# MatchaChoco010/toy-cpu-pathtracing

Measured on AMD Instinct MI355X. Metric: Msamples/sec (whole node), scene3 MIS/Sobol 1920x1080, higher is better.
Workload: dtype f32; 1 GPU; scene3 1920x1080 mis+sobol, 1024-spp job, 1024 sample indices per step (BASELINE configs[1]); parallelism=single-gpu

## Files before the change

toy-cpu-pathtracing_amd/csrc/api.cpp:

```cpp
#include <cstring>

#include "api_internal.hpp"

using namespace pt;

static thread_local std::string g_err;
bool pt::g_debug_unlocked = false;
int pt::fail(int code, const std::string& msg) { g_err = msg; return code; }

static const uint32_t CIE_CMF_BITS[470 * 4] = {
#include "cie_cmf.inc"
};
void pt::cie_cmf4(float out[470 * 4]) { std::memcpy(out, CIE_CMF_BITS, sizeof(CIE_CMF_BITS)); }

int pt::get_launch_ctx(const mi355pt_scene* sc, uint32_t seed, LaunchCtx** out, int* slot) {
    if (sc->ctx && sc->ctx->device != sc->impl.device) {
        delete sc->ctx; sc->ctx = nullptr;
    }
    if (!sc->ctx) {
        LaunchCtx* lc = new LaunchCtx();
        lc->device = sc->impl.device;
        HIP_TRY(hipMalloc((void**)&lc->d_hash, sizeof(uint64_t) * HASH_TABLE_DIMS));
        HIP_TRY(hipMalloc((void**)&lc->d_counters, sizeof(unsigned) * CTX_RING));
        HIP_TRY(hipMalloc((void**)&lc->d_stats, sizeof(DevStats) * CTX_RING));
// ... 78 lines not shown
    if (hipGetDevice(&dev) != hipSuccess || dev != s->impl.device)
        return fail(MI355PT_E_DEVICE, "current HIP device is not the device the scene was built on");
    return MI355PT_OK;
}

static int launch_range(const mi355pt_scene* s, const mi355pt_camera* cam, const mi355pt_params* p, uint32_t s_begin, uint32_t s_end, float* d_accum,
                        hipStream_t stream, mi355pt_stats* stats, const PathOut& pout, int aov_kind, uint32_t illuminant_lut, const uint32_t* d_list,
                        uint32_t n_list) {
    const bool aov = aov_kind >= 0;
    if (!d_list && shard_tile_count(cam->width, cam->height, p->shard_index, p->shard_count) == 0) return MI355PT_OK;
    int rc;
    LaunchCtx* lc; int slot;
    if ((rc = get_launch_ctx(s, p->seed, &lc, &slot))) return rc;
    if (lc->device != s->impl.device) return fail(MI355PT_E_DEVICE, "launch context and scene live on different devices");
    const bool want_stats = stats && p->collect_stats;
    int& waves = aov ? lc->aov_waves[aov_kind] : lc->waves[want_stats ? 1 : 0][p->sampler & 1u][p->strategy < 3u ? p->strategy : 0u];
    if (!waves) waves = aov ? query_resident_waves_aov((uint32_t)aov_kind, s->impl.features)
                            : query_resident_waves(select_kernel(false, want_stats, s->impl.features, p->sampler, p->strategy));
    const DevCamera dc = make_camera(cam);
    LaunchPlan plan = d_list ? plan_launch_tiles(cam, p, s_begin, s_end, waves, n_list) : plan_launch(cam, p, s_begin, s_end, waves, aov);
    DevParams& dp = plan.params;
    if (d_list) set_tile_list(dp, d_list);
    dp.stats_mode = p->collect_stats;
    return timed_launch(lc, slot, stream, stats, want_stats || aov, [&](unsigned* d_counter, DevStats* d_stats) {
        if ((rc = grow_device_buffer(&lc->d_partial, &lc->partial_bytes, plan.partial_floats * sizeof(float), stream))) return rc;
        const KernelKey key = select_kernel(d_list != nullptr, want_stats, s->impl.features, p->sampler, p->strategy);
        if ((rc = grow_device_buffer(&lc->d_defer, &lc->defer_bytes, aov ? (size_t)0 : query_defer_bytes_per_wave(key) * (size_t)plan.grid, stream))) return rc;
        if (aov) HIP_TRY(launch_aov((uint32_t)aov_kind, s->impl.dev, dc, dp, illuminant_lut, lc->d_hash, d_accum, d_counter, stats ? d_stats : nullptr,
                                    s->impl.features, plan.grid, stream));
        else {
            DevScene dev = s->impl.dev;
            dev.cam_lists = use_camera_lists(key, dp.block_log2, camera_lists_enabled()) ? 1u : 0u;
            dev.queue_stage = use_queue_staging(key, queue_staging_enabled()) ? 1u : 0u;
            dev.light_queue = use_light_queue(key, light_queue_enabled()) ? 1u : 0u;
            HIP_TRY(launch_pt(key, dev, dc, dp, plan.n_tiles,
                              lc->d_hash, d_accum, lc->d_partial, d_counter, d_list ? nullptr : d_stats, plan.grid, stream, pout, lc->d_defer));
        }
        return (int)MI355PT_OK;
    });
}

int pt::launch_ranges(const mi355pt_scene* s, const mi355pt_camera* cam, const mi355pt_params* p, uint32_t s_begin, uint32_t s_end, float* d_accum,
                      hipStream_t stream, mi355pt_stats* stats, const uint32_t* d_list, uint32_t n_list, const PathOut& pout, int aov_kind,
                      uint32_t illuminant_lut) {
    return for_each_launch_range(p->sampler, stats != nullptr, s_begin, s_end, [&](uint32_t b, uint32_t e) {
        return launch_range(s, cam, p, b, e, d_accum, stream, stats, pout, aov_kind, illuminant_lut, d_list, n_list);
    });
}

int pt::render_accum_range(const mi355pt_scene* s, const mi355pt_camera* cam, const mi355pt_params* p, uint32_t s_begin, uint32_t s_end,
                           float* d_accum, void* hip_stream, mi355pt_stats* stats, const PathOut& pout, int aov_kind, uint32_t illuminant_lut) {
    const bool aov = aov_kind >= 0;
    int rc = check_args(s, cam, p, aov);
    if (rc) return rc;
    if (!d_accum || s_end > p->spp || s_begin >= s_end) return fail(MI355PT_E_INVALID, "bad sample range or null accumulator");
    if (aov) {
        if (aov_kind > MI355PT_AOV_SHADING_NORMAL) return fail(MI355PT_E_INVALID, "unknown AOV kind");
        if (p->collect_stats) return fail(MI355PT_E_INVALID, "the AOV renderers have no instrumented kernel: collect_stats must be 0");
        if (aov_kind == MI355PT_AOV_ALBEDO && illuminant_lut >= s->impl.luts.size())
// ... 95 lines not shown
```

toy-cpu-pathtracing_amd/csrc/launch_plan.hpp:

```cpp
#pragma once
#include <algorithm>
#include <cmath>
#include <cstddef>
#include <cstdint>
#include <cstdlib>

#include "../../include/mi355pt.h"
#include "layout.hpp"

namespace pt {

struct V3 { float x, y, z; };
inline V3 cross3(V3 a, V3 b) { return {a.y * b.z - b.y * a.z, a.z * b.x - b.z * a.x, a.x * b.y - b.x * a.y}; }
inline V3 norm3(V3 a) { float r = 1.0f / std::sqrt((a.x * a.x) + (a.y * a.y) + (a.z * a.z)); return {a.x * r, a.y * r, a.z * r}; }

inline uint32_t log2_int(uint32_t v) { return v == 0 ? 0 : 31 - (uint32_t)__builtin_clz(v); }
inline uint32_t round_up_pow2(uint32_t v) { return v <= 1 ? 1 : 1u << (32 - __builtin_clz(v - 1)); }

inline uint32_t shard_tile_count(uint32_t width, uint32_t height, uint32_t shard_index, uint32_t shard_count) {
    const uint32_t total = ((width + 7) / 8) * ((height + 7) / 8);
    const uint32_t cnt = shard_count ? shard_count : 1u, idx = shard_count ? shard_index : 0u;
    return total > idx ? (total - idx + cnt - 1) / cnt : 0u;
}

// ... 136 lines not shown
#undef PT_SET_ENTRY
inline uint32_t pick_features(uint32_t feat) {
    for (uint32_t s : FEATURE_SETS) if ((feat & ~s) == 0u) return s;
    return FEAT_ALL;
}
struct KernelKey { bool tiles, stats; uint32_t mode, set; };
inline KernelKey select_kernel(bool tiles, bool stats, uint32_t feat, uint32_t sampler, uint32_t strategy) {
    if (stats) return KernelKey{tiles, true, MODE_GENERIC, (feat & (FEAT_CC | FEAT_EMTEX)) == 0u ? FEAT_STD & ~FEAT_CC : FEAT_ALL};
    const uint32_t mode = sampler == MI355PT_SAMPLER_SOBOL && strategy == MI355PT_STRATEGY_MIS ? MODE_MIS_SOBOL
                        : sampler == MI355PT_SAMPLER_SOBOL && strategy == MI355PT_STRATEGY_NEE ? MODE_NEE_SOBOL
                        : strategy == MI355PT_STRATEGY_PT ? MODE_PT : MODE_GENERIC;
    return KernelKey{tiles, false, mode, pick_features(feat)};
}

inline bool use_camera_lists(const KernelKey& key, uint32_t block_log2, bool enabled) { return enabled && !key.stats && block_log2 <= 3u; }
inline bool camera_lists_enabled() { const char* e = getenv("MI355PT_NO_CAMERA_LISTS"); return !(e && e[0] != '\0' && !(e[0] == '0' && e[1] == '\0')); }

inline bool use_queue_staging(const KernelKey& key, bool enabled) { return enabled && !key.stats; }
inline bool queue_staging_enabled() { const char* e = getenv("MI355PT_NO_QUEUE_STAGING"); return !(e && e[0] != '\0' && !(e[0] == '0' && e[1] == '\0')); }

inline bool use_light_queue(const KernelKey& key, bool enabled) { return enabled && !key.stats; }
inline bool light_queue_enabled() { const char* e = getenv("MI355PT_NO_LIGHT_QUEUE"); return !(e && e[0] != '\0' && !(e[0] == '0' && e[1] == '\0')); }

}
```

toy-cpu-pathtracing_amd/csrc/layout.hpp:

```cpp
#pragma once
#include <stddef.h>
#include <stdint.h>

#if defined(__HIPCC__)
#define PT_HD __host__ __device__
#else
#define PT_HD
#endif

namespace pt {

#ifndef PT_STACK_DEPTH
#define PT_STACK_DEPTH 24
#endif
constexpr int STACK_DEPTH = PT_STACK_DEPTH;
constexpr int MAX_LEAF_TRIS = 4;
constexpr int MAX_BUILD_DEPTH = 22;
constexpr int HASH_TABLE_DIMS = 136;

struct alignas(16) DevNode {
    float bx[4];
    float by[4];
    float bz[4];
    int32_t child[2];
// ... 139 lines not shown
    const DevTri* tris_render;
    float tri_shift[3]; uint32_t tris_are_local;
    float shared_mw[3]; uint32_t pad_mw;
    const DevInstance* instances;
    const DevMaterial* materials;
    const DevLight* lights;
    const DevLightTri* light_tris;
    const float* light_uvs;
    const float* luts;
    const float* cmf;
    const float* rgb2spec;
    const float* z_nodes;
    const uint32_t* texels;
    const DevTexture* textures;
    const float* cc_albedo;
    uint32_t n_nodes, n_tris, n_lights, n_materials;
    int32_t root;
    int32_t root4;
    uint32_t n_nodes4;
    uint32_t cam_lists;
    const DevEnv* envs;
    uint32_t n_envs;
    uint16_t queue_stage;
    uint16_t light_queue;
};

struct DevCamera {
    float s[3], u[3], f[3];
    float tan_half_fov, aspect;
    uint32_t width, height;
};

struct DevParams {
    uint32_t spp, seed, max_depth, strategy, sampler;
    float exposure;
    uint32_t log2_spp, n_base4_digits;
    uint32_t sample_begin, sample_end;
    uint32_t shard_index, shard_count;
    uint32_t tiles_x, tiles_y;
    uint32_t n_work;
    uint32_t chunks, chunk_size;
    uint32_t block_log2;
    uint32_t sample_prefix_digits;
    uint32_t stats_mode;
    uint32_t albedo_lut;
    float rr_gate;
    float xyz_to_rgb[9];
// ... 21 lines not shown
```

toy-cpu-pathtracing_amd/csrc/pt_kernel_body.inc:

```
    __shared__ __attribute__((aligned(16))) uint32_t s_stack[STACK_DEPTH * 64];
#ifndef PT_FILM_PIX
#define PT_FILM_PIX 64
#endif
    __shared__ float s_film[PT_FILM_PIX * 3];
    __shared__ uint32_t s_hi[SOBOL_HI_DIMS];
    __shared__ uint32_t s_p6[SOBOL_HI_DIMS];
    __shared__ unsigned s_work;
    constexpr bool PARK = (FEAT & FEAT_CC) != 0u && kernel_min_waves<FEAT>() <= 3;
    __shared__ float s_park[PARK ? 8 * 64 : 1];
    __shared__ uint8_t s_perm[96];
    __shared__ uint32_t s_ring[ANY_RING];
    __shared__ uint32_t s_occl[2];
    __shared__ uint32_t s_pair[64];
    const AnyLds any_lds{s_ring, s_occl, s_pair};
    __shared__ unsigned long long s_best[64];
    const ClosestLds closest_lds{s_ring, s_best, s_pair};
    __shared__ uint32_t s_infl[2];
    const PairLds pair_lds{s_ring, s_best, s_occl, s_pair, s_infl};
    constexpr bool CAMLIST = !STATS && tail_queue<FEAT, MODE>();
    __shared__ uint32_t s_cand[CAMLIST ? CAM_LIST_CAP : 1u];
    DevParams prm = prm_in;
    if constexpr (MODE == MODE_MIS_SOBOL) { prm.strategy = 2u; prm.sampler = 1u; }
    if constexpr (MODE == MODE_NEE_SOBOL) { prm.strategy = 1u; prm.sampler = 1u; }
    if constexpr (MODE == MODE_PT) prm.strategy = 0u;
// ... 6 lines not shown
                s_park[4 * 64 + lane] = Q.p_pdf; s_park[5 * 64 + lane] = Q.prev_pos.x; s_park[6 * 64 + lane] = Q.prev_pos.y; s_park[7 * 64 + lane] = Q.prev_pos.z;
            }
#pragma unroll
            for (int i = 0; i < 4; ++i) Q.pf[i] = 0.0f;
            Q.p_pdf = 0.0f; Q.prev_pos = mk3(0.0f, 0.0f, 0.0f);
        }
    };
    auto unpark = [&](Path& Q) {
        if constexpr (PARK) {
#pragma unroll
            for (int i = 0; i < 4; ++i) Q.pf[i] = s_park[i * 64 + lane];
            Q.p_pdf = s_park[4 * 64 + lane]; Q.prev_pos = mk3(s_park[5 * 64 + lane], s_park[6 * 64 + lane], s_park[7 * 64 + lane]);
        }
    };
    uint32_t* stack = s_stack + lane;
    for (uint32_t k = lane; k < 96u; k += 64u) s_perm[k] = (uint8_t)((perm_packed(k >> 2) >> (2u * (k & 3u))) & 3u);
    if constexpr ((FEAT & (FEAT_TEX | FEAT_EMTEX | FEAT_ENV)) != 0u) s_znodes[lane] = sc.z_nodes[lane];
    __syncthreads();
    SamplerCtx sctx{prm.sampler, prm.seed, prm.log2_spp, prm.n_base4_digits, cam.width, dim_hash_tab, nullptr, 0u, 0u, nullptr, s_perm};
    StatCounters st{};
    unsigned long long tp[10] = {0, 0, 0, 0, 0, 0, 0, 0, 0, 0};
    unsigned long long dvc[8] = {0, 0, 0, 0, 0, 0, 0, 0};
    unsigned long long t_loop0 = 0;
    if (STATS) t_loop0 = __builtin_amdgcn_s_memtime();

    for (;;) {
        if (lane == 0) s_work = atomicAdd(work_counter, 1u);
        __syncthreads();
        const uint32_t work = s_work;
        __syncthreads();
        if (work >= prm.n_work) break;
        const LaneJob job = PT_LANE_JOB(work, lane, cam, prm);
        const LaneJob job0 = PT_LANE_JOB(work, 0u, cam, prm);
        const uint32_t blk_log2 = prm.block_log2, blk_mask = (1u << blk_log2) - 1u;
        const uint32_t s_prefix = prm.sample_prefix_digits;
        const uint32_t hi_first_w = sobol_hi_first(prm.log2_spp, blk_log2) - s_prefix, hi_shift_w = 2u * hi_first_w - (prm.log2_spp & 1u);
        if (prm.sampler == 1u && hi_first_w < prm.n_base4_digits && hi_first_w >= 3u &&
            2u * prm.n_base4_digits - (prm.log2_spp & 1u) <= hi_shift_w + 27u) {
            sctx.hi_first = sobol_hi_first(prm.log2_spp, blk_log2) - s_prefix;
            sctx.hi_shift = 2u * sctx.hi_first - (prm.log2_spp & 1u);
            const uint32_t tile_m = (encode_morton2_u32(job0.px, job0.py) << prm.log2_spp) | (s_prefix ? job0.s_cur : 0u);
            for (uint32_t dmn = lane; dmn < (uint32_t)SOBOL_HI_DIMS; dmn += 64) {
                uint32_t e = (uint32_t)(sobol_tile_hi_digits(tile_m, dmn, prm.log2_spp, prm.n_base4_digits, sctx.hi_first) >> sctx.hi_shift);
                const uint64_t prefix = (uint64_t)tile_m >> sctx.hi_shift;
                e |= sobol_perm_index(prefix, dmn) << 27;
                uint32_t e6 = 0;
// ... 179 lines not shown
                    const uint32_t tile_k = (work / prm.chunks) >> (6u - 2u * blk_log2);
                    const uint32_t smp_i = P.smp.morton & ((1u << prm.log2_spp) - 1u);
                    sample_log(P, pout, ((size_t)tile_k * 64u + ((py & 7u) * 8u + (px & 7u))) * pout.n_s + (smp_i - pout.s_base));
                }
                float r, g, b;
                film_rgb(P, sc, prm, r, g, b);
                atomicAdd(&s_film[3 * my_pix], r); atomicAdd(&s_film[3 * my_pix + 1], g); atomicAdd(&s_film[3 * my_pix + 2], b);
            };
            if constexpr (TAILQ) {
                bool end_path = dying;
                const bool front = active && !dying && !susp;
                unpark(P);
                bool lq_push = false, lq_void = false;
                if constexpr (LIGHTQ) {
                    const bool on_emitter = front && got && (hit.mclass & 7u) == MT_EMISSIVE;
                    lq_void = on_emitter && emitter_hit_is_void<STATS>(prm, P.from_camera, P.prev_spec);
                    lq_push = on_emitter && !lq_void;
                }
                const unsigned long long m_lq = (LIGHTQ && sc.light_queue != 0u) ? __ballot(lq_push) : 0ull;
                {
                    ShadeCtx C0;
                    C0.cont = false;
                    if constexpr (LIGHTQ) {
                        if (front && !lq_push && !lq_void) end_path = shade_vertex_head<STATS, FEAT, 3>(P, sc, prm, sctx, got, hit, sh, st, tsa, C0);
                        if (lq_void) end_path = true;
                    } else {
                        if (front) end_path = shade_vertex_head<STATS, FEAT, 1>(P, sc, prm, sctx, got, hit, sh, st, tsa, C0);
                    }
                }
                dying = false;
                const bool go_on = front && !lq_push && !end_path;
                const bool cls2 = TQ_CLASSES != 0u && ((TQ_CLASSES >> (hit.mclass & 31u)) & 1u) != 0u;
                const unsigned long long m_on1 = __ballot(go_on && !cls2), m_on2 = TQ_CLASSES != 0u ? __ballot(go_on && cls2) : 0ull;
                uint32_t n_on1 = 0u;
                bool stage = false;
                if constexpr (STAGE) {
                    n_on1 = (uint32_t)__popcll(m_on1);
                    stage = sc.queue_stage != 0u && tq_stage_pushes(q_count, n_on1, pool_next >= pool_size, (uint32_t)PT_TAILQ_MIN);
                }
                if ((m_on1 | m_on2 | m_lq) != 0ull) {
                    if constexpr (LIGHTQ) {
                        if (lq_push && m_lq != 0ull) {
                            lq_put(lq_base + (lq_push_slot(lq_count, rank_below(m_lq)) & (LQ_SLOTS - 1u)), P, hit, my_pix);
                            active = false;
                        }
                        lq_count += (uint32_t)__popcll(m_lq);
                    }
// ... 32 lines not shown
                            lq_count -= n;
                        }
                    }
                    if (ev) {
                        emitter_hit<STATS, FEAT>(sc, prm, hit, P.rd, P.T, P.pf, P.p_pdf, P.prev_pos, P.wl, P.from_camera, P.prev_spec, P.L, st);
                        finish_path();
                        active = false;
                    }
                }
                if (STATS) ts3 = ts4 = __builtin_amdgcn_s_memtime();
                const bool draining = pool_next >= pool_size;
                if (tq_pass_due(q_count, q2_count, draining, TQ_CLASSES != 0u, (uint32_t)PT_TAILQ_MIN)) {
                    const unsigned long long m_free = __ballot(!active);
                    const uint32_t n_free = (uint32_t)__popcll(m_free), r = rank_below(m_free);
                    const TqTake tk = tq_pass_take(q_count, q2_count, n_free, draining, TQ_CLASSES != 0u, (uint32_t)PT_TAILQ_MIN);
                    const uint32_t n2 = tk.n2, n1 = tk.n1;
                    const bool take2 = !active && r < n2, take1 = !active && !take2 && r - n2 < n1;
                    const bool take = take1 || take2;
                    const uint32_t e = take2 ? QUEUE_RING + tq_pop_slot(q2_count, n2, r) : tq_pop_slot(q_count, n1, r - n2);
                    TqStagePop sp{0u, false, 0u};
                    if constexpr (STAGE) sp = tq_stage_pop(stage ? q_count - n_on1 : q_count, stage ? n_on1 : 0u, n1, r - n2);
                    q2_count -= n2; q_count -= n1;
                    bool ep = false;
                    if constexpr ((FEAT & FEAT_CC) != 0u) {
                        ShadeCtx C;
                        shade_ctx_idle_cc(C);
                        if (take) {
                            __builtin_amdgcn_fence(__ATOMIC_ACQUIRE, "workgroup");
                            tq_load(e, P, hit, my_pix);
                            active = true;
                            shade_vertex_head<STATS, FEAT, 2>(P, sc, prm, sctx, true, hit, sh, st, tsa, C);
                        }
                        const bool want_mc = take && C.cont && C.need_cc;
                        const float fc_mc = coat_directional_albedo_coop(want_mc, C.cc_alpha_c, C.cc_r0c, C.wo_nm, C.mc_key, lane);
                        if (want_mc) C.cc_fc = fc_mc;
                        if (take && C.cont) ep = shade_vertex_tail<STATS, FEAT>(P, sc, prm, sctx, sh, st, tsb, C);
                    } else if (take) {
                        __builtin_amdgcn_fence(__ATOMIC_ACQUIRE, "workgroup");
                        static_assert(STAGE, "the kernels without the clearcoat code have one queue");
                        TqRec rec;
                        if (!sp.staged) rec = tq_get(q_base + sp.slot, QR);
                        else rec = tq_get(s_stage + sp.index, TQ_STAGE_SLOTS);
                        tq_unpack(rec, P, hit, my_pix);
                        active = true;
                        ShadeCtx C;
                        C.cont = false; C.need_cc = false; C.cc_fc = 0.0f;
                        shade_vertex_head<STATS, FEAT, 2>(P, sc, prm, sctx, true, hit, sh, st, tsa, C);
                        if (C.cont) ep = shade_vertex_tail<STATS, FEAT>(P, sc, prm, sctx, sh, st, tsb, C);
                    }
                    park(P, take);
                    if (sh.on && sh.c[0] == 0.0f && sh.c[1] == 0.0f && sh.c[2] == 0.0f && sh.c[3] == 0.0f) sh.on = false;
                    if (!active) sh.on = false;
                    if (take) { dying = sh.on && ep; if (dying) ep = false; }
                    if (take && ep) { finish_path(); active = false; }
                }
            } else
            for (int pass = 0;; ++pass) {
            const bool mine = pass == 0 || popped;
            bool end_path = pass == 0 && MERGED && dying;
            if (pass == 0) {
                if constexpr (!MERGED) sh = ShadowReq{};
                unpark(P);
            }
            if constexpr (DEFER != 0u) {
                if (popped) {
                    __builtin_amdgcn_fence(__ATOMIC_ACQUIRE, "workgroup");
                    dq_load(pop_e, P, hit, my_pix);
                    got = true;
                }
                const bool defer_now = pass == 0 && !(STATS && prm.stats_mode == 1u) && active && !dying && !susp && !popped && got && ((DEFER >> (hit.mclass & 31u)) & 1u) != 0u;
                const unsigned long long m_def = __ballot(defer_now);
                if (m_def != 0ull) {
                    if (defer_now) {
                        dq_store((q_tail + rank_below(m_def)) & (DEFER_RING - 1u), P, hit, my_pix);
                        active = false;
                    }
// ... 72 lines not shown
                tp[0] += ts1 - ts0; tp[1] += ts2 - ts1; tp[2] += ts3 - ts2; tp[3] += ts4 - ts3; tp[4] += ts5 - ts4;
                if (tsa) { tp[6] += tsa - ts2; if (tsb) { tp[7] += tsb - tsa; tp[8] += ts3 - tsb; } else tp[7] += ts3 - tsa; } else tp[6] += ts3 - ts2;
            }
        }
        __syncthreads();
        if (job.valid) {
            size_t o = ((size_t)job.py * cam.width + job.px) * 3;
            const float fr = s_film[3 * lane], fg = s_film[3 * lane + 1], fb = s_film[3 * lane + 2];
            if (prm.chunks == 1) { accum[o] += fr; accum[o + 1] += fg; accum[o + 2] += fb; }
            else {
                const uint32_t tile_k = (work / prm.chunks) >> (6u - 2u * blk_log2), chunk = work % prm.chunks;
                float* slot = partial + (((size_t)tile_k * prm.chunks + chunk) * 64u + ((job.py & 7u) * 8u + (job.px & 7u))) * 3u;
                slot[0] = fr; slot[1] = fg; slot[2] = fb;
            }
        }
        __syncthreads();
    }
    if (STATS && lane == 0) {
        tp[5] = __builtin_amdgcn_s_memtime() - t_loop0;
        for (int i = 0; i < 10; ++i) atomicAdd(&stats->phase_cycles[i], tp[i]);
        for (int i = 0; i < 8; ++i) atomicAdd(&stats->divergence[4 + i], dvc[i]);
    }
    if (STATS) flush_stats(stats, st);
```

toy-cpu-pathtracing_amd/csrc/pt_path.hpp:

```cpp
#pragma once
#include "launch.hpp"
#include "pt_device.hpp"
#include "pt_ggx.hpp"

namespace pt {

constexpr float RAY_EPS = 1e-5f;
constexpr float SHADOW_EPS = 1e-4f;

struct Frame { f3 t, b, n; };
PT_DEV f3 to_local(const Frame& f, f3 v) { return mk3(dot(f.t, v), dot(f.b, v), dot(f.n, v)); }
PT_DEV f3 to_world(const Frame& f, f3 v) { return f.t * v.x + f.b * v.y + f.n * v.z; }
PT_DEV Frame shading_frame(f3 shading_normal, f3 tangent) {
    Frame f;
    f.n = normalize(shading_normal);
    f.b = normalize(cross(normalize(f.n), tangent));
    f.t = normalize(cross(f.b, f.n));
    return f;
}
#ifndef PT_EXACT_DIV
#define PT_EXACT_DIV 0
#endif
#ifndef PT_FRAME_INVERSE
#define PT_FRAME_INVERSE 2
// ... 364 lines not shown
                    }
                    for (uint32_t li = 0; li < sc.n_lights; ++li) {
                        DevLight lt = sc.lights[li];
                        if (lt.kind != LK_ENV) continue;
                        const DevMaterial* lm = sc.materials + lt.material;
                        float ph[4];
                        DevSpectrum ls = load_spectrum(&lm->color);
                        eval_spectrum<false, (FEAT & FEAT_EMTEX) != 0, (FEAT & FEAT_EMTEX) != 0>(sc, ls, wl, f2{0.5f, 0.5f}, ph, st);
                        float sum = 0.0f;
#pragma unroll
                        for (int i = 0; i < 4; ++i) sum += (ph[i] * lm->intensity_avg) * lt.area_sum;
                        const float probability = inf_sum == 0.0f ? 0.0f : (sum / 4.0f) / inf_sum;
                        light_pdf += probability * env_pdf(sc.envs[lt.first_tri], rd);
                    }
                }
                float w = balance_heuristic(p_pdf, light_pdf);
                float tf = 1.0f / p_pdf;
#pragma unroll
                for (int i = 0; i < 4; ++i) L[i] = L[i] + ((((T[i] * pf[i]) * rad[i]) * tf) * w);
            }
        }
    } else {
        Surface sf; const DevMaterial* mat = nullptr; uint32_t mtype;
        if (PHASE == 1 || PHASE == 3) {
            mtype = hit.mclass & 7u;
            if (PHASE == 1 && mtype == MT_EMISSIVE) { sf = load_surface(sc, hit, rd); mat = sc.materials + sf.material; }
        } else { sf = load_surface(sc, hit, rd); mat = sc.materials + sf.material; mtype = mat->type; }
        const bool emissive = PHASE != 2 && PHASE != 3 && mtype == MT_EMISSIVE;
        float Le[4] = {0, 0, 0, 0};
        if constexpr (PHASE != 2) {
        if (emissive) {
            DevSpectrum rs = load_spectrum(&mat->color);
            eval_spectrum<STATS, (FEAT & FEAT_EMTEX) != 0, (FEAT & FEAT_EMTEX) != 0>(sc, rs, wl, sf.uv, Le, st);
            float inten = mat->intensity;
            if ((FEAT & FEAT_EMTEX) && mat->metallic_tex != 0xffffffffu) { float t3[3]; bilinear_rgb(sc, mat->metallic_tex, sf.uv, t3); inten = t3[0]; }
#pragma unroll
            for (int i = 0; i < 4; ++i) Le[i] = Le[i] * inten;
        }
        if (from_camera) {
            if (emissive) {
#pragma unroll
                for (int i = 0; i < 4; ++i) L[i] = L[i] + T[i] * Le[i];
            }
        } else {
            float tf = 1.0f / p_pdf;
            if (emissive) {
                float w = 1.0f;
                if (prm.strategy == 1u) w = prev_spec ? 1.0f : 0.0f;
                else if (prm.strategy == 2u && !prev_spec) {
                    float wsum = 0.0f, wme = 0.0f;
                    if (!(FEAT & FEAT_MLIGHT) || sc.n_lights == 1u) {
// ... 24 lines not shown
                        float wt = sum / 4.0f;
                        wsum += wt;
                        if (li == sf.light) wme = wt;
                    }
                    float probability = wsum == 0.0f ? 0.0f : wme / wsum;
                    f3 dv = prev_pos - sf.p;
                    float distance = length(dv);
                    f3 wo_l = -normalize(dv);
                    float pdf_dir = sf.light_pdf_area * (distance * distance) / fabsf(dot(sf.ng, wo_l));
                    w = balance_heuristic(p_pdf, probability * pdf_dir);
                }
                if (w != 0.0f || prm.strategy != 1u) {
#pragma unroll
                    for (int i = 0; i < 4; ++i) L[i] = L[i] + (T[i] * ((pf[i] * Le[i]) * tf)) * w;
                }
            } else if (prm.strategy != 1u || prev_spec) {
                float w = (prm.strategy == 2u && !prev_spec) ? balance_heuristic(p_pdf, 0.0f) : 1.0f;
#pragma unroll
                for (int i = 0; i < 4; ++i) L[i] = L[i] + (T[i] * 0.0f) * w;
            }
#pragma unroll
            for (int i = 0; i < 4; ++i) T[i] = T[i] * (pf[i] * tf);
            float p = fmaxf(fmaxf(fmaxf(fmaxf(-INFINITY, T[0]), T[1]), T[2]), T[3]);
            if (!(p >= prm.rr_gate)) {
                float ur = get_1d(smp, sctx);
                if (ur < p) {
                    if (p != 0.0f) {
#pragma unroll
                        for (int i = 0; i < 4; ++i) T[i] = T[i] / p;
                    }
                } else end_path = true;
            }
        }
        if (!end_path) {
            depth += 1;
            if (depth > prm.max_depth || emissive) end_path = true;
        }
        }
        if (PHASE != 1 && PHASE != 3 && !end_path) {
            if (STATS) { st.bounces++; tsa = __builtin_amdgcn_s_memtime(); }
            Frame fr, fw_num;
            if constexpr (numeric_frames<FEAT>()) shading_frames_numeric(sf.ns, sf.tangent, fr, fw_num);
            else fr = shading_frame(sf.ns, sf.tangent);
            const Frame& fw = numeric_frames<FEAT>() ? fw_num : fr;
            f3 wo_r = sf.wo;
            f3 wo = to_local(fr, wo_r);
            f3 ng_t = normalize(to_local(fw, sf.ng));
            const bool is_diel = (FEAT & FEAT_DIEL) && (mtype == MT_GLASS || mtype == MT_PLASTIC);
            float uc = 0.0f;
            f2 uv = f2{0.0f, 0.0f};
            float d_alpha = mat->roughness;
            if ((FEAT & FEAT_TEX) && (FEAT & FEAT_ROUGH) && is_diel && mat->roughness_tex != 0xffffffffu) { float t3[3]; bilinear_rgb(sc, mat->roughness_tex, sf.uv, t3); d_alpha = t3[0]; }
            const bool rough_diel = (FEAT & FEAT_ROUGH) && is_diel && d_alpha >= 1e-3f;
            if (is_diel) {
                uc = get_1d(smp, sctx);
                if (rough_diel || (mtype == MT_PLASTIC && mat->color.kind == SPK_TEXTURE)) uv = get_2d(smp, sctx); else smp.dimension += 2;
            }
            else if ((FEAT & FEAT_CC) && mtype == MT_CLEARCOAT) { uc = get_1d(smp, sctx); uv = get_2d(smp, sctx); }
            else { smp.dimension += 1; uv = get_2d(smp, sctx); }
            Frame nf, nfw_num;
            if ((FEAT & FEAT_TEX) && mat->normal_tex != 0xffffffffu) {
                float rgb[3];
// ... 627 lines not shown
```

toy-cpu-pathtracing_amd/csrc/scene.cpp:

```cpp
#include "scene.hpp"

#include <hip/hip_runtime.h>

#include <chrono>
#include <cstdlib>
#include <cstring>

#include "scene_lower.hpp"

namespace pt {

namespace {

template <typename T>
int upload_array(SceneImpl* s, const std::vector<T>& v, const T** out, std::string* err) {
    void* p = nullptr;
    size_t bytes = std::max<size_t>(v.size() * sizeof(T), 16);
    hipError_t e = hipMalloc(&p, bytes);
    if (e != hipSuccess) { *err = std::string("hipMalloc: ") + hipGetErrorString(e); return MI355PT_E_DEVICE; }
    s->allocs.push_back(p);
    if (!v.empty()) {
        e = hipMemcpy(p, v.data(), v.size() * sizeof(T), hipMemcpyHostToDevice);
        if (e != hipSuccess) { *err = std::string("hipMemcpy: ") + hipGetErrorString(e); return MI355PT_E_DEVICE; }
    }
    *out = (const T*)p;
    return MI355PT_OK;
}

double ms_since(std::chrono::steady_clock::time_point t0) { return std::chrono::duration<double, std::milli>(std::chrono::steady_clock::now() - t0).count(); }

// ... 3 lines not shown
void SceneImpl::release() {
    for (void* p : allocs) (void)hipFree(p);
    allocs.clear();
    rebase = RebaseState{};
    built = false;
}

int SceneImpl::upload(const LoweredScene& ls, std::string* err) {
    int rc;
    dev = ls.dev;
    if ((rc = upload_array(this, ls.nodes, &dev.nodes, err))) return rc;
#if PT_NODE_Q16
    if ((rc = upload_array(this, ls.nodes4, &dev.nodes4q, err))) return rc;
#else
    if ((rc = upload_array(this, ls.nodes4, &dev.nodes4, err))) return rc;
#endif
    if ((rc = upload_array(this, ls.tris_render, &dev.tris_render, err))) return rc;
    if ((rc = upload_array(this, ls.shade, &dev.shade, err))) return rc;
    if ((rc = upload_array(this, ls.instances, &dev.instances, err))) return rc;
    if ((rc = upload_array(this, ls.tris_local, &dev.tris_local, err))) return rc;
    dev.tris = dev.tris_are_local ? dev.tris_local : dev.tris_render;
    if ((rc = upload_array(this, ls.cc_albedo, &dev.cc_albedo, err))) return rc;
    if ((rc = upload_array(this, ls.materials, &dev.materials, err))) return rc;
    if ((rc = upload_array(this, ls.lights, &dev.lights, err))) return rc;
    if ((rc = upload_array(this, ls.light_tris, &dev.light_tris, err))) return rc;
    if ((rc = upload_array(this, ls.light_uvs, &dev.light_uvs, err))) return rc;
    if ((rc = upload_array(this, ls.luts, &dev.luts, err))) return rc;
    if ((rc = upload_array(this, ls.cmf, &dev.cmf, err))) return rc;
    if ((rc = upload_array(this, ls.rgb2spec, &dev.rgb2spec, err))) return rc;
    if ((rc = upload_array(this, ls.z_nodes, &dev.z_nodes, err))) return rc;
    if ((rc = upload_array(this, ls.texels, &dev.texels, err))) return rc;
    if ((rc = upload_array(this, ls.textures, &dev.textures, err))) return rc;
    std::vector<DevEnv> envs = ls.envs;
    for (size_t ek = 0; ek < envs.size(); ++ek) {
        if ((rc = upload_array(this, ls.env_tables[ek].texels, &envs[ek].texels, err))) return rc;
        if ((rc = upload_array(this, ls.env_tables[ek].marginal, &envs[ek].marginal, err))) return rc;
        if ((rc = upload_array(this, ls.env_tables[ek].conditional, &envs[ek].conditional, err))) return rc;
    }
    return upload_array(this, envs, &dev.envs, err);
}

int SceneImpl::build(const mi355pt_camera* cam, const float* cmf4 , std::string* err) {
    release();
    int ndev = 0, rc;
    if (hipGetDeviceCount(&ndev) != hipSuccess || ndev == 0) { *err = "no HIP device: the product path requires a gfx950 GPU"; return MI355PT_E_NO_DEVICE; }
    (void)hipGetDevice(&device);
    std::memcpy(build_cam_pos, cam->position, sizeof(build_cam_pos));
// ... 45 lines not shown
```

toy-cpu-pathtracing_amd/csrc/scene_lower.cpp:

```cpp
#include "scene_lower.hpp"

#include <algorithm>
#include <cfloat>
#include <cmath>
#include <cstdio>
#include <cstring>

#include "instance_move_plan.hpp"

namespace pt {

namespace {

constexpr float PI_F = 3.14159265358979323846f;

struct V3 { float x, y, z; };
inline V3 operator-(V3 a, V3 b) { return {a.x - b.x, a.y - b.y, a.z - b.z}; }
inline V3 cross(V3 a, V3 b) { return {a.y * b.z - b.y * a.z, a.z * b.x - b.z * a.x, a.x * b.y - b.x * a.y}; }
inline float dot(V3 a, V3 b) { return (a.x * b.x) + (a.y * b.y) + (a.z * b.z); }
inline float length(V3 a) { return std::sqrt(dot(a, a)); }
inline V3 normalize(V3 a) { float r = 1.0f / length(a); return {a.x * r, a.y * r, a.z * r}; }
inline V3 vertex(const HostMesh& mesh, uint32_t v) { return V3{mesh.pos[3 * v], mesh.pos[3 * v + 1], mesh.pos[3 * v + 2]}; }
inline bool degenerate(V3 a, V3 b, V3 c) { const V3 cr = cross(b - a, c - a); return dot(cr, cr) == 0.0f; }

// ... 693 lines not shown
           " depth=" + std::to_string(rep.bvh_depth) + " builder=" + (gpu_builder ? "gpu" : "host") + t_bvh + " collapse=" + rep.collapse_method + t_collapse + tail;
}

void lowering_digests(const LoweredScene& ls, const LowerReport& rep, std::vector<std::string>* names, std::vector<uint64_t>* digests) {
    names->clear(); digests->clear();
    auto add = [&](const std::string& name, const void* p, size_t bytes) { names->push_back(name); digests->push_back(fnv1a64(p, bytes)); };
#define PT_DIGEST(v) add(#v, ls.v.data(), ls.v.size() * sizeof(ls.v[0]))
    PT_DIGEST(nodes); PT_DIGEST(nodes4); PT_DIGEST(tris_render); PT_DIGEST(shade); PT_DIGEST(instances); PT_DIGEST(tris_local); PT_DIGEST(cc_albedo);
    PT_DIGEST(materials); PT_DIGEST(lights); PT_DIGEST(light_tris); PT_DIGEST(light_uvs); PT_DIGEST(luts); PT_DIGEST(cmf); PT_DIGEST(rgb2spec);
    PT_DIGEST(z_nodes); PT_DIGEST(texels); PT_DIGEST(textures);
#undef PT_DIGEST
    for (size_t k = 0; k < ls.env_tables.size(); ++k) {
        const LoweredScene::EnvTables& t = ls.env_tables[k];
        const std::string e = "env" + std::to_string(k);
        add(e + ".texels", t.texels.data(), t.texels.size() * 4); add(e + ".marginal", t.marginal.data(), t.marginal.size() * 4);
        add(e + ".conditional", t.conditional.data(), t.conditional.size() * 4);
    }
    add("envs", ls.envs.data(), ls.envs.size() * sizeof(DevEnv));
    std::string b;
    auto put = [&](const void* p, size_t n) { b.append((const char*)p, n); };
    const DevScene& dev = ls.dev;
    put(dev.grid_org, 12); put(dev.grid_cell, 12); put(dev.tri_shift, 12); put(&dev.tris_are_local, 4); put(dev.shared_mw, 12); put(&dev.pad_mw, 4);
    put(&dev.n_nodes, 4); put(&dev.n_tris, 4); put(&dev.n_lights, 4); put(&dev.n_materials, 4); put(&dev.root, 4); put(&dev.root4, 4);
    put(&dev.n_nodes4, 4); put(&dev.cam_lists, 4); put(&dev.n_envs, 4); put(&dev.queue_stage, 2); put(&dev.light_queue, 2);
    const uint32_t feat = ls.features; const uint64_t ndeg = rep.n_degenerate, nn4 = dev.n_nodes4; const int32_t depth = rep.bvh_depth, need = rep.stack_need;
    put(&feat, 4); put(&ndeg, 8); put(&depth, 4); put(&nn4, 8); put(&need, 4); put(rep.collapse_method, std::strlen(rep.collapse_method));
    add("scalars", b.data(), b.size());
}

}
```

toy-cpu-pathtracing_amd/csrc/scene_update.cpp:

```cpp
#include "scene_update.hpp"

namespace pt {

SceneUpdateResult scene_update_step(SceneImpl* impl, const SceneUpdate& u) {
    SceneUpdateResult r;
    auto dropped = [&](const char* what, hipError_t e) { impl->release(); r.outcome = SceneUpdateResult::DEVICE_ERROR; r.what = std::string(what) + ": " + hipGetErrorString(e); return r; };
#define STEP_TRY(what, expr) do { const hipError_t _e = (expr); if (_e != hipSuccess) return dropped(what, _e); } while (0)
#if PT_NODE_Q16
    return dropped("scene_update_step", hipErrorNotSupported);
#else
    RebaseState& rb = impl->rebase;
    DevScene& d = impl->dev;
    hipStream_t stream = nullptr;
    const size_t n_inst = impl->instances.size(), n_pdf = u.light_pdf ? u.light_pdf->size() : 0;
    const bool has_tree = u.sah && d.root >= 0 && rb.n_entries > 0;

    if (u.moved) { STEP_TRY("hipMalloc", ensure(impl, &rb.d_moved_bits, (n_inst + 31) / 32)); STEP_TRY("hipMalloc", ensure(impl, &rb.d_light_pdf, n_pdf)); }
    if (u.sah) STEP_TRY("hipMalloc", ensure(impl, &rb.d_sah, sah_scratch_floats(rb.n_entries)));
    if (u.deform) { STEP_TRY("hipMalloc", ensure(impl, &rb.d_deform_staging, u.deform->staging_capacity)); STEP_TRY("hipMalloc", ensure(impl, &rb.d_deform_table, u.deform->table_capacity)); }
    if (u.deform) STEP_TRY("hipMalloc", ensure(impl, &rb.d_mesh_idx, rb.mesh_idx_offset.back()));
    if (u.sah && !rb.sah_built_valid) {
        rb.sah_built = 0.0f;
        if (has_tree) {
            STEP_TRY("launch_sah_cost", launch_sah_cost(d.nodes, d.root, rb.d_entries, rb.n_entries, rb.d_sah, stream));
            STEP_TRY("hipMemcpy", hipMemcpy(&rb.sah_built, rb.d_sah, sizeof(float), hipMemcpyDeviceToHost));
        }
        rb.sah_built_valid = true;
    }
    if (u.deform) {
        for (const DeformUpdate& m : u.deform->meshes) {
            if (rb.mesh_idx_uploaded[m.geom]) continue;
            STEP_TRY("hipMemcpy", hipMemcpy(rb.d_mesh_idx + rb.mesh_idx_offset[m.geom], impl->meshes[m.geom].idx.data(), (size_t)3 * m.n_tri * sizeof(uint32_t), hipMemcpyHostToDevice));
            rb.mesh_idx_uploaded[m.geom] = 1;
        }
        STEP_TRY("hipMemcpy", hipMemcpy(rb.d_deform_staging, u.deform->staging.data(), u.deform->staging.size() * sizeof(float), hipMemcpyHostToDevice));
        STEP_TRY("hipMemcpy", hipMemcpy(rb.d_deform_table, u.deform->table.data(), u.deform->table.size() * sizeof(uint32_t), hipMemcpyHostToDevice));
    }

    STEP_TRY("hipMemcpy", hipMemcpy((void*)d.instances, u.rec.instances.data(), u.rec.instances.size() * sizeof(DevInstance), hipMemcpyHostToDevice));
    if (!u.rec.lights.empty()) STEP_TRY("hipMemcpy", hipMemcpy((void*)d.lights, u.rec.lights.data(), u.rec.lights.size() * sizeof(DevLight), hipMemcpyHostToDevice));
    if (!u.rec.light_tris.empty()) STEP_TRY("hipMemcpy", hipMemcpy((void*)d.light_tris, u.rec.light_tris.data(), u.rec.light_tris.size() * sizeof(DevLightTri), hipMemcpyHostToDevice));
    if (u.moved) {
        std::vector<uint32_t> bits((n_inst + 31) / 32, 0u);
        for (size_t i = 0; i < n_inst; ++i) if (u.moved[i]) bits[i >> 5] |= 1u << (i & 31u);
        STEP_TRY("hipMemcpy", hipMemcpy(rb.d_moved_bits, bits.data(), bits.size() * sizeof(uint32_t), hipMemcpyHostToDevice));
        if (n_pdf) STEP_TRY("hipMemcpy", hipMemcpy(rb.d_light_pdf, u.light_pdf->data(), n_pdf * sizeof(float), hipMemcpyHostToDevice));
    }
    STEP_TRY("hipMemset", hipMemset(rb.d_count, 0, sizeof(uint32_t)));
    Event ev_a, ev_b;
    STEP_TRY("hipEventCreate", ev_a.create()); STEP_TRY("hipEventCreate", ev_b.create());
    STEP_TRY("hipEventRecord", ev_a.record(stream));
    if (u.deform) {
        STEP_TRY("launch_deform_tris", launch_deform_tris((DevTriLocal*)d.tris_local, (DevTriShade*)d.shade, rb.d_deform_table, rb.d_deform_staging, rb.d_mesh_idx, d.n_tris,
                                                          (uint32_t)n_inst, (uint32_t)deform_table_slots_at(n_inst), u.deform->n_slots, stream));
        ++r.launches;
    }
    STEP_TRY("launch_rebase_tris", launch_rebase_tris(d.tris_local, d.instances, (DevTri*)d.tris_render, d.n_tris, u.count_degenerate, rb.d_count, stream));
    ++r.launches;
    if (u.moved) {
        STEP_TRY("launch_shade_refresh", launch_shade_refresh((DevTriShade*)d.shade, d.tris_local, d.instances, rb.d_moved_bits, d.lights, rb.d_light_pdf, d.n_tris, (uint32_t)n_inst,
                                                              d.n_lights, (uint32_t)n_pdf, stream));
        ++r.launches;
    }
    for (size_t h = 0; h + 1 < rb.height_offset.size(); ++h) {
// ... 32 lines not shown
```

Measured before the change: 2801 Msamples/s.

## Decide Russian roulette early and skip tracing rays that cannot reach a light

Moves the Russian-roulette termination decision ahead of tracing the next bounce. A path that is doomed to end, with no environment map and no emitter box its ray could hit, is ended right away instead of tracing a ray whose hit would add nothing. Per-light AABBs with padding are stored after the light array and kept up to date by scene updates. The light-queue head shading uses a new phase that honours the doomed bit. This adds a loop over all lights for each doomed path, and it changes the order in which sampler dimensions are drawn.

```diff
diff --git a/toy-cpu-pathtracing_amd/csrc/api.cpp b/toy-cpu-pathtracing_amd/csrc/api.cpp
--- a/toy-cpu-pathtracing_amd/csrc/api.cpp
+++ b/toy-cpu-pathtracing_amd/csrc/api.cpp
@@ -124,7 +124,8 @@
     DevParams& dp = plan.params;
     if (d_list) set_tile_list(dp, d_list);
     dp.stats_mode = p->collect_stats;
-    return timed_launch(lc, slot, stream, stats, want_stats || aov, [&](unsigned* d_counter, DevStats* d_stats) {
+    const bool count_ends = stats && !want_stats && !aov && g_debug_unlocked;
+    return timed_launch(lc, slot, stream, stats, want_stats || aov || count_ends, [&](unsigned* d_counter, DevStats* d_stats) {
         if ((rc = grow_device_buffer(&lc->d_partial, &lc->partial_bytes, plan.partial_floats * sizeof(float), stream))) return rc;
         const KernelKey key = select_kernel(d_list != nullptr, want_stats, s->impl.features, p->sampler, p->strategy);
         if ((rc = grow_device_buffer(&lc->d_defer, &lc->defer_bytes, aov ? (size_t)0 : query_defer_bytes_per_wave(key) * (size_t)plan.grid, stream))) return rc;
@@ -135,8 +136,9 @@
             dev.cam_lists = use_camera_lists(key, dp.block_log2, camera_lists_enabled()) ? 1u : 0u;
             dev.queue_stage = use_queue_staging(key, queue_staging_enabled()) ? 1u : 0u;
             dev.light_queue = use_light_queue(key, light_queue_enabled()) ? 1u : 0u;
+            dev.early_path_end = use_early_path_end(key, early_path_end_enabled()) ? 1u : 0u;
             HIP_TRY(launch_pt(key, dev, dc, dp, plan.n_tiles,
-                              lc->d_hash, d_accum, lc->d_partial, d_counter, d_list ? nullptr : d_stats, plan.grid, stream, pout, lc->d_defer));
+                              lc->d_hash, d_accum, lc->d_partial, d_counter, (want_stats && !d_list) || count_ends ? d_stats : nullptr, plan.grid, stream, pout, lc->d_defer));
         }
         return (int)MI355PT_OK;
     });
diff --git a/toy-cpu-pathtracing_amd/csrc/launch_plan.hpp b/toy-cpu-pathtracing_amd/csrc/launch_plan.hpp
--- a/toy-cpu-pathtracing_amd/csrc/launch_plan.hpp
+++ b/toy-cpu-pathtracing_amd/csrc/launch_plan.hpp
@@ -182,4 +182,7 @@
 inline bool use_light_queue(const KernelKey& key, bool enabled) { return enabled && !key.stats; }
 inline bool light_queue_enabled() { const char* e = getenv("MI355PT_NO_LIGHT_QUEUE"); return !(e && e[0] != '\0' && !(e[0] == '0' && e[1] == '\0')); }
 
+inline bool use_early_path_end(const KernelKey& key, bool enabled) { return enabled && !key.stats; }
+inline bool early_path_end_enabled() { const char* e = getenv("MI355PT_NO_EARLY_PATH_END"); return !(e && e[0] != '\0' && !(e[0] == '0' && e[1] == '\0')); }
+
 }
diff --git a/toy-cpu-pathtracing_amd/csrc/layout.hpp b/toy-cpu-pathtracing_amd/csrc/layout.hpp
--- a/toy-cpu-pathtracing_amd/csrc/layout.hpp
+++ b/toy-cpu-pathtracing_amd/csrc/layout.hpp
@@ -185,7 +185,8 @@
     const DevEnv* envs;
     uint32_t n_envs;
     uint16_t queue_stage;
-    uint16_t light_queue;
+    uint8_t light_queue;
+    uint8_t early_path_end;
 };
 
 struct DevCamera {
diff --git a/toy-cpu-pathtracing_amd/csrc/path_end_plan.hpp b/toy-cpu-pathtracing_amd/csrc/path_end_plan.hpp
--- /dev/null
+++ b/toy-cpu-pathtracing_amd/csrc/path_end_plan.hpp
@@ -0,0 +1,87 @@
+#pragma once
+#include <cstdint>
+#include <vector>
+
+#include "layout.hpp"
+
+namespace pt {
+
+constexpr uint32_t PATH_DOOMED_BIT = 0x80000000u;
+
+PT_HD inline float pe_max(float a, float b) { return a < b ? b : a; }
+PT_HD inline float pe_min(float a, float b) { return b < a ? b : a; }
+PT_HD inline float pe_abs(float v) { return v < 0.0f ? -v : v; }
+PT_HD inline float pe_fmax(float a, float b) { return (b != b) ? a : ((a != a) ? b : (a < b ? b : a)); }
+
+PT_HD inline float path_end_pmax(const float T[4], const float pf[4], float p_pdf) {
+    const float tf = 1.0f / p_pdf;
+    float p = -__builtin_huge_valf();
+    for (int i = 0; i < 4; ++i) p = pe_fmax(p, T[i] * (pf[i] * tf));
+    return p;
+}
+PT_HD inline bool path_end_draws(float p, float rr_gate) { return !(p >= rr_gate); }
+PT_HD inline bool path_end_doomed(float p, float ur, float rr_gate, uint32_t depth, uint32_t max_depth) {
+    if (path_end_draws(p, rr_gate) && !(ur < p)) return true;
+    return depth + 1u > max_depth;
+}
+
+PT_HD inline bool path_end_term_is_zero(const float T[4], float w) {
+    bool zero = true;
+    for (int i = 0; i < 4; ++i) zero = zero && ((T[i] * 0.0f) * w == 0.0f);
+    return zero;
+}
+
+constexpr uint32_t LIGHT_BOX_FLOATS = 8u;
+constexpr float LIGHT_BOX_PAD = 1.0f / 16384.0f;
+PT_HD inline float light_box_host_pad(const float lo[3], const float hi[3], const float shift[3]) {
+    float m = 0.0f, s = 0.0f;
+    for (int a = 0; a < 3; ++a) { m = pe_max(m, pe_max(pe_abs(lo[a]), pe_abs(hi[a]))); s = pe_max(s, pe_abs(shift[a])); }
+    return LIGHT_BOX_PAD * (m + s);
+}
+PT_HD inline bool light_box_may_reach(const float o[3], const float d[3], const float lo[3], const float hi[3], float pad_host) {
+    if (!(lo[0] <= hi[0])) return false;
+    const float pad = pad_host + LIGHT_BOX_PAD * pe_max(pe_abs(o[0]), pe_max(pe_abs(o[1]), pe_abs(o[2])));
+    if (!(pad == pad)) return true;
+    float tn = 0.0f, tf = __builtin_huge_valf();
+    for (int a = 0; a < 3; ++a) {
+        const float inv = 1.0f / d[a];
+        const float t0 = ((lo[a] - pad) - o[a]) * inv, t1 = ((hi[a] + pad) - o[a]) * inv;
+        if (!(t0 == t0) || !(t1 == t1)) return true;
+        tn = pe_max(tn, pe_min(t0, t1)); tf = pe_min(tf, pe_max(t0, t1));
+    }
+    return !(tn > tf);
+}
+
+inline void light_boxes(const std::vector<DevLight>& lights, const std::vector<DevLightTri>& light_tris, const float shift[3], std::vector<float>* out) {
+    out->assign(lights.size() * LIGHT_BOX_FLOATS, 0.0f);
+    for (size_t li = 0; li < lights.size(); ++li) {
+        float lo[3] = {1.0f, 1.0f, 1.0f}, hi[3] = {-1.0f, -1.0f, -1.0f};
+        const DevLight& l = lights[li];
+        if (l.kind == LK_AREA && l.n_tris != 0u && (size_t)l.first_tri + l.n_tris <= light_tris.size()) {
+            for (int a = 0; a < 3; ++a) { lo[a] = __builtin_huge_valf(); hi[a] = -__builtin_huge_valf(); }
+            for (uint32_t t = 0; t < l.n_tris; ++t) {
+                const DevLightTri& r = light_tris[l.first_tri + t];
+                const float v[3][3] = {{r.p0[0], r.p0[1], r.p0[2]}, {r.p1x, r.p1yz[0], r.p1yz[1]}, {r.p2xy[0], r.p2xy[1], r.p2z}};
+                for (int k = 0; k < 3; ++k) for (int a = 0; a < 3; ++a) { lo[a] = pe_min(lo[a], v[k][a]); hi[a] = pe_max(hi[a], v[k][a]); }
+            }
+        }
+        float* b = out->data() + li * LIGHT_BOX_FLOATS;
+        b[0] = lo[0]; b[1] = lo[1]; b[2] = lo[2]; b[3] = (lo[0] <= hi[0]) ? light_box_host_pad(lo, hi, shift) : 0.0f;
+        b[4] = hi[0]; b[5] = hi[1]; b[6] = hi[2]; b[7] = 0.0f;
+    }
+}
+inline size_t light_allocation_bytes(size_t n_lights) { return n_lights * (sizeof(DevLight) + LIGHT_BOX_FLOATS * sizeof(float)); }
+inline std::vector<unsigned char> light_allocation(const std::vector<DevLight>& lights, const std::vector<DevLightTri>& light_tris, const float shift[3]) {
+    std::vector<float> boxes;
+    light_boxes(lights, light_tris, shift, &boxes);
+    std::vector<unsigned char> bytes(light_allocation_bytes(lights.size()));
+    unsigned char* p = bytes.data();
+    for (size_t i = 0; i < lights.size() * sizeof(DevLight); ++i) p[i] = ((const unsigned char*)lights.data())[i];
+    for (size_t i = 0; i < boxes.size() * sizeof(float); ++i) p[lights.size() * sizeof(DevLight) + i] = ((const unsigned char*)boxes.data())[i];
+    return bytes;
+}
+PT_HD inline const float* light_box_of(const DevLight* lights, uint32_t n_lights, uint32_t li) {
+    return (const float*)(lights + n_lights) + (size_t)li * LIGHT_BOX_FLOATS;
+}
+
+}
diff --git a/toy-cpu-pathtracing_amd/csrc/pt_kernel_body.inc b/toy-cpu-pathtracing_amd/csrc/pt_kernel_body.inc
--- a/toy-cpu-pathtracing_amd/csrc/pt_kernel_body.inc
+++ b/toy-cpu-pathtracing_amd/csrc/pt_kernel_body.inc
@@ -52,6 +52,7 @@
     unsigned long long tp[10] = {0, 0, 0, 0, 0, 0, 0, 0, 0, 0};
     unsigned long long dvc[8] = {0, 0, 0, 0, 0, 0, 0, 0};
     unsigned long long t_loop0 = 0;
+    uint32_t n_early = 0u;
     if (STATS) t_loop0 = __builtin_amdgcn_s_memtime();
 
     for (;;) {
@@ -277,7 +278,7 @@
                     ShadeCtx C0;
                     C0.cont = false;
                     if constexpr (LIGHTQ) {
-                        if (front && !lq_push && !lq_void) end_path = shade_vertex_head<STATS, FEAT, 3>(P, sc, prm, sctx, got, hit, sh, st, tsa, C0);
+                        if (front && !lq_push && !lq_void) end_path = shade_vertex_head<STATS, FEAT, 4>(P, sc, prm, sctx, got, hit, sh, st, tsa, C0);
                         if (lq_void) end_path = true;
                     } else {
                         if (front) end_path = shade_vertex_head<STATS, FEAT, 1>(P, sc, prm, sctx, got, hit, sh, st, tsa, C0);
@@ -356,6 +357,7 @@
                     if constexpr (STAGE) sp = tq_stage_pop(stage ? q_count - n_on1 : q_count, stage ? n_on1 : 0u, n1, r - n2);
                     q2_count -= n2; q_count -= n1;
                     bool ep = false;
+                    bool ended_early = false;
                     if constexpr ((FEAT & FEAT_CC) != 0u) {
                         ShadeCtx C;
                         shade_ctx_idle_cc(C);
@@ -381,11 +383,33 @@
                         C.cont = false; C.need_cc = false; C.cc_fc = 0.0f;
                         shade_vertex_head<STATS, FEAT, 2>(P, sc, prm, sctx, true, hit, sh, st, tsa, C);
                         if (C.cont) ep = shade_vertex_tail<STATS, FEAT>(P, sc, prm, sctx, sh, st, tsb, C);
-                    }
+                        if (C.cont && !ep) {
+                            const float p_next = path_end_pmax(P.T, P.pf, P.p_pdf);
+                            float ur = 0.0f;
+                            if (path_end_draws(p_next, prm.rr_gate)) ur = get_1d(P.smp, sctx);
+                            if (path_end_doomed(p_next, ur, prm.rr_gate, P.depth, prm.max_depth)) {
+                                P.depth |= PATH_DOOMED_BIT;
+                                bool skip = sc.early_path_end != 0u && sc.n_envs == 0u;
+                                if (skip && !emitter_hit_is_void<STATS>(prm, false, P.prev_spec)) {
+                                    const float w = (prm.strategy == 2u && !P.prev_spec) ? balance_heuristic(P.p_pdf, 0.0f) : 1.0f;
+                                    skip = path_end_term_is_zero(P.T, w);
+                                    const float o[3] = {P.ro.x, P.ro.y, P.ro.z}, d[3] = {P.rd.x, P.rd.y, P.rd.z};
+                                    for (uint32_t li = 0u; li < sc.n_lights; ++li) {
+                                        const float4* bx = (const float4*)light_box_of(sc.lights, sc.n_lights, li);
+                                        const float4 b0 = bx[0], b1 = bx[1];
+                                        const float lo[3] = {b0.x, b0.y, b0.z}, hi[3] = {b1.x, b1.y, b1.z};
+                                        if (light_box_may_reach(o, d, lo, hi, b0.w)) skip = false;
+                                    }
+                                }
+                                if (skip) { ep = true; ended_early = true; }
+                            }
+                        }
+                    }
+                    if constexpr (STAGE) n_early += (uint32_t)__popcll(__ballot(ended_early));
                     park(P, take);
                     if (sh.on && sh.c[0] == 0.0f && sh.c[1] == 0.0f && sh.c[2] == 0.0f && sh.c[3] == 0.0f) sh.on = false;
                     if (!active) sh.on = false;
-                    if (take) { dying = sh.on && ep; if (dying) ep = false; }
+                    if (take) { dying = (sh.on && ep) || ended_early; if (dying) ep = false; }
                     if (take && ep) { finish_path(); active = false; }
                 }
             } else
@@ -504,3 +528,4 @@
         for (int i = 0; i < 8; ++i) atomicAdd(&stats->divergence[4 + i], dvc[i]);
     }
     if (STATS) flush_stats(stats, st);
+    if (!STATS && n_early != 0u && stats != nullptr && lane == 0) atomicAdd(&stats->wave_steps[7], (unsigned long long)n_early);
diff --git a/toy-cpu-pathtracing_amd/csrc/pt_path.hpp b/toy-cpu-pathtracing_amd/csrc/pt_path.hpp
--- a/toy-cpu-pathtracing_amd/csrc/pt_path.hpp
+++ b/toy-cpu-pathtracing_amd/csrc/pt_path.hpp
@@ -1,5 +1,6 @@
 #pragma once
 #include "launch.hpp"
+#include "path_end_plan.hpp"
 #include "pt_device.hpp"
 #include "pt_ggx.hpp"
 
@@ -410,11 +411,11 @@
         }
     } else {
         Surface sf; const DevMaterial* mat = nullptr; uint32_t mtype;
-        if (PHASE == 1 || PHASE == 3) {
+        if (PHASE == 1 || PHASE == 3 || PHASE == 4) {
             mtype = hit.mclass & 7u;
             if (PHASE == 1 && mtype == MT_EMISSIVE) { sf = load_surface(sc, hit, rd); mat = sc.materials + sf.material; }
         } else { sf = load_surface(sc, hit, rd); mat = sc.materials + sf.material; mtype = mat->type; }
-        const bool emissive = PHASE != 2 && PHASE != 3 && mtype == MT_EMISSIVE;
+        const bool emissive = PHASE != 2 && PHASE != 3 && PHASE != 4 && mtype == MT_EMISSIVE;
         float Le[4] = {0, 0, 0, 0};
         if constexpr (PHASE != 2) {
         if (emissive) {
@@ -485,6 +486,13 @@
 #pragma unroll
             for (int i = 0; i < 4; ++i) T[i] = T[i] * (pf[i] * tf);
             float p = fmaxf(fmaxf(fmaxf(fmaxf(-INFINITY, T[0]), T[1]), T[2]), T[3]);
+            if constexpr (PHASE == 4) {
+                if ((depth & PATH_DOOMED_BIT) != 0u) end_path = true;
+                else if (!(p >= prm.rr_gate) && p != 0.0f) {
+#pragma unroll
+                    for (int i = 0; i < 4; ++i) T[i] = T[i] / p;
+                }
+            } else
             if (!(p >= prm.rr_gate)) {
                 float ur = get_1d(smp, sctx);
                 if (ur < p) {
@@ -500,7 +508,7 @@
             if (depth > prm.max_depth || emissive) end_path = true;
         }
         }
-        if (PHASE != 1 && PHASE != 3 && !end_path) {
+        if (PHASE != 1 && PHASE != 3 && PHASE != 4 && !end_path) {
             if (STATS) { st.bounces++; tsa = __builtin_amdgcn_s_memtime(); }
             Frame fr, fw_num;
             if constexpr (numeric_frames<FEAT>()) shading_frames_numeric(sf.ns, sf.tangent, fr, fw_num);
diff --git a/toy-cpu-pathtracing_amd/csrc/scene.cpp b/toy-cpu-pathtracing_amd/csrc/scene.cpp
--- a/toy-cpu-pathtracing_amd/csrc/scene.cpp
+++ b/toy-cpu-pathtracing_amd/csrc/scene.cpp
@@ -6,6 +6,7 @@
 #include <cstdlib>
 #include <cstring>
 
+#include "path_end_plan.hpp"
 #include "scene_lower.hpp"
 
 namespace pt {
@@ -55,7 +56,12 @@
     dev.tris = dev.tris_are_local ? dev.tris_local : dev.tris_render;
     if ((rc = upload_array(this, ls.cc_albedo, &dev.cc_albedo, err))) return rc;
     if ((rc = upload_array(this, ls.materials, &dev.materials, err))) return rc;
-    if ((rc = upload_array(this, ls.lights, &dev.lights, err))) return rc;
+    {
+        const std::vector<unsigned char> bytes = light_allocation(ls.lights, ls.light_tris, ls.dev.tri_shift);
+        const unsigned char* p = nullptr;
+        if ((rc = upload_array(this, bytes, &p, err))) return rc;
+        dev.lights = (const DevLight*)p;
+    }
     if ((rc = upload_array(this, ls.light_tris, &dev.light_tris, err))) return rc;
     if ((rc = upload_array(this, ls.light_uvs, &dev.light_uvs, err))) return rc;
     if ((rc = upload_array(this, ls.luts, &dev.luts, err))) return rc;
diff --git a/toy-cpu-pathtracing_amd/csrc/scene_lower.cpp b/toy-cpu-pathtracing_amd/csrc/scene_lower.cpp
--- a/toy-cpu-pathtracing_amd/csrc/scene_lower.cpp
+++ b/toy-cpu-pathtracing_amd/csrc/scene_lower.cpp
@@ -739,7 +739,7 @@
     const DevScene& dev = ls.dev;
     put(dev.grid_org, 12); put(dev.grid_cell, 12); put(dev.tri_shift, 12); put(&dev.tris_are_local, 4); put(dev.shared_mw, 12); put(&dev.pad_mw, 4);
     put(&dev.n_nodes, 4); put(&dev.n_tris, 4); put(&dev.n_lights, 4); put(&dev.n_materials, 4); put(&dev.root, 4); put(&dev.root4, 4);
-    put(&dev.n_nodes4, 4); put(&dev.cam_lists, 4); put(&dev.n_envs, 4); put(&dev.queue_stage, 2); put(&dev.light_queue, 2);
+    put(&dev.n_nodes4, 4); put(&dev.cam_lists, 4); put(&dev.n_envs, 4); put(&dev.queue_stage, 2); put(&dev.light_queue, 1); put(&dev.early_path_end, 1);
     const uint32_t feat = ls.features; const uint64_t ndeg = rep.n_degenerate, nn4 = dev.n_nodes4; const int32_t depth = rep.bvh_depth, need = rep.stack_need;
     put(&feat, 4); put(&ndeg, 8); put(&depth, 4); put(&nn4, 8); put(&need, 4); put(rep.collapse_method, std::strlen(rep.collapse_method));
     add("scalars", b.data(), b.size());
diff --git a/toy-cpu-pathtracing_amd/csrc/scene_update.cpp b/toy-cpu-pathtracing_amd/csrc/scene_update.cpp
--- a/toy-cpu-pathtracing_amd/csrc/scene_update.cpp
+++ b/toy-cpu-pathtracing_amd/csrc/scene_update.cpp
@@ -1,4 +1,6 @@
 #include "scene_update.hpp"
+
+#include "path_end_plan.hpp"
 
 namespace pt {
 
@@ -37,9 +39,16 @@
         STEP_TRY("hipMemcpy", hipMemcpy(rb.d_deform_table, u.deform->table.data(), u.deform->table.size() * sizeof(uint32_t), hipMemcpyHostToDevice));
     }
 
+    if (!u.rec.lights.empty() && u.rec.lights.size() != (size_t)d.n_lights) return dropped("scene_update_step: light list changed since the build", hipErrorInvalidValue);
     STEP_TRY("hipMemcpy", hipMemcpy((void*)d.instances, u.rec.instances.data(), u.rec.instances.size() * sizeof(DevInstance), hipMemcpyHostToDevice));
     if (!u.rec.lights.empty()) STEP_TRY("hipMemcpy", hipMemcpy((void*)d.lights, u.rec.lights.data(), u.rec.lights.size() * sizeof(DevLight), hipMemcpyHostToDevice));
     if (!u.rec.light_tris.empty()) STEP_TRY("hipMemcpy", hipMemcpy((void*)d.light_tris, u.rec.light_tris.data(), u.rec.light_tris.size() * sizeof(DevLightTri), hipMemcpyHostToDevice));
+    if (!u.rec.lights.empty()) {
+        const float zero[3] = {0.0f, 0.0f, 0.0f};
+        std::vector<float> boxes;
+        light_boxes(u.rec.lights, u.rec.light_tris, u.rec.tris_are_local ? u.rec.shared_iw : zero, &boxes);
+        STEP_TRY("hipMemcpy", hipMemcpy((void*)light_box_of(d.lights, d.n_lights, 0u), boxes.data(), boxes.size() * sizeof(float), hipMemcpyHostToDevice));
+    }
     if (u.moved) {
         std::vector<uint32_t> bits((n_inst + 31) / 32, 0u);
         for (size_t i = 0; i < n_inst; ++i) if (u.moved[i]) bits[i >> 5] |= 1u << (i & 31u);
```

Result: faster. 2897 Msamples/s (median of 6 runs) (+3.4%).
